# yabebalFantaye/MCEvidence

Hardware: AMD Instinct MI355X
Metric: knn_queries_per_sec (higher is better)
Workload: dtype f16 filter + f64 refine (exact f64 results)

## Files before the change

mcevidence_amd/csrc/capi_common.hpp:

```cpp
#pragma once
namespace {

thread_local char g_err[512] = "";
thread_local char g_last_kernel[256] = "";
thread_local int g_prof_on = 0;
thread_local std::vector<std::pair<hipEvent_t, hipEvent_t>> g_ev_pool;
thread_local size_t g_ev_used = 0;
thread_local size_t g_ev_calls = 0;
thread_local bool g_in_tail = false;
thread_local int g_split_depth = 0;
thread_local double g_last_prune_geom[3] = {0, 0, 0};
thread_local double g_last_flops_main = 0.0, g_last_flops_all = 0.0;
thread_local std::vector<std::pair<hipEvent_t, hipEvent_t>> g_evs_pool;
thread_local size_t g_evs_used = 0;

int fail(int code, const char* fmt, ...)
{
    va_list ap;
    va_start(ap, fmt);
    vsnprintf(g_err, sizeof(g_err), fmt, ap);
    va_end(ap);
    return code;
}

#define MCE_HIP(call)                                                                              \
    do {                                                                                           \
        hipError_t e_ = (call);                                                                    \
        if (e_ != hipSuccess)                                                                      \
            return fail(MCE_ERR_HIP, "%s failed: %s (%s:%d)", #call, hipGetErrorString(e_), __FILE__, __LINE__); \
    } while (0)

std::atomic<int> g_mode{0};
std::atomic<int> g_prune_mode{0};
struct Tuning {
    bool sym_kernel_f16 = false, tail_split = true, prune_prof = false, wide = true;
    int spin_limit = 1 << 21, sym_bucket = 0, sym_panel = 0, sym_seed_rows = 0, sym_seed_share = 2, sym_seed_mode = -1;
    int f16_seed_rows = -1, f16_seed_share = -1, f16_seed_tg = -1, rsplit = 0, panel_debug = 0, sym_chains = 0, panel_qt = 0;
    size_t feed_wave_bytes = 0;
};
Tuning read_tuning()
{
    Tuning t;
    auto num = [](const char* name, int dflt) { const char* e = getenv(name); return e ? atoi(e) : dflt; };
    const char* e = getenv("MCE_SYM_KERNEL");
    t.sym_kernel_f16 = e && strcmp(e, "f16") == 0;
    t.spin_limit = num("MCE_SYM_SPIN_LIMIT", 1 << 21);
    t.sym_bucket = num("MCE_SYM_BUCKET", 0);
    t.sym_panel = num("MCE_SYM_PANEL", 0);
    t.sym_chains = num("MCE_SYM_CHAINS", 0);
    t.sym_seed_rows = num("MCE_SYM_SEED_ROWS", 0);
    t.sym_seed_share = num("MCE_SYM_SEED_SHARE", 2);
    t.sym_seed_mode = num("MCE_SYM_SEED_MODE", -1);
    t.f16_seed_rows = num("MCE_F16_SEED_ROWS", -1);
    t.f16_seed_share = num("MCE_F16_SEED_SHARE", -1);
    t.f16_seed_tg = num("MCE_F16_SEED_TG", -1);
    t.rsplit = num("MCE_RSPLIT", 0);
    t.tail_split = num("MCE_TAIL_SPLIT", 1) != 0;
    t.wide = num("MCE_WIDE", 1) != 0;
    t.panel_debug = num("MCE_PANEL_DEBUG", 0);
    t.panel_qt = num("MCE_PANEL_QT", 0);
    t.prune_prof = getenv("MCE_PRUNE_PROF") != nullptr;
    if ((e = getenv("MCE_FEED_WAVE_BYTES"))) t.feed_wave_bytes = (size_t)std::strtoull(e, nullptr, 10);
    return t;
}
std::atomic<int> g_sym_mode{-1};
int sym_mode()
{
    int m = g_sym_mode.load();
    if (m < 0) {
        const char* e = getenv("MCE_SYM");
        m = e ? atoi(e) : 0;
        if (m < 0 || m > 2) m = 0;
        g_sym_mode.store(m);
    }
    return m;
}
const char* env_prune_heavy() { return getenv("MCE_PRUNE_HEAVY"); }
const char* env_prune_lists() { return getenv("MCE_PRUNE_LISTS"); }
const char* env_prune_times() { return getenv("MCE_PRUNE_TIMES"); }
bool env_long_on() { static const bool v = [] { const char* e = getenv("MCE_LONG"); return !(e && e[0] == '0'); }(); return v; }
bool env_deep_on() { static const bool v = [] { const char* e = getenv("MCE_DEEP"); return !(e && e[0] == '0'); }(); return v; }
int env_feed_eig() { static const int v = [] { const char* e = getenv("MCE_FEED_EIG"); return e && !strcmp(e, "hip") ? 2 : 1; }(); return v; }
bool env_feed_upload_async() { static const bool v = [] { const char* e = getenv("MCE_FEED_UPLOAD"); return e && !strcmp(e, "async"); }(); return v; }
int env_pairs_once_split() { static const int v = [] { const char* e = getenv("MCE_PAIRS_ONCE_SPLIT"); const int n = e ? atoi(e) : 0; return (n >= 1 && n <= 8) ? n : 0; }(); return v; }
int env_pairs_once_panel() { static const int v = [] { const char* e = getenv("MCE_PAIRS_ONCE_PANEL"); const int n = e ? atoi(e) : 0; return n >= 1 ? n : 0; }(); return v; }
struct CallOptions { int search = -1, prune = -1, sym = -1, same_set = -1, verify = -1, eig = 0; };
thread_local CallOptions t_opt;
thread_local std::vector<CallOptions> t_opt_stack;
int eff_search_mode() { return t_opt.search >= 0 ? t_opt.search : g_mode.load(); }
int eff_prune_mode() { return t_opt.prune >= 0 ? t_opt.prune : g_prune_mode.load(); }
int eff_sym_mode() { return t_opt.sym >= 0 ? t_opt.sym : sym_mode(); }
constexpr int kVerifyDefaultRows = 256;
constexpr int64_t kVerifyAlwaysFrom = 65536;
// ... 4 lines not shown
        const char* e = getenv("MCE_VERIFY");
        if (!e || !*e) return kVerifyDefaultRows;
        const long n = strtol(e, nullptr, 10);
        return (int)std::max<long>(0, std::min<long>(n, 1 << 20));
    }();
    return v;
}
bool verify_env_set() { static const bool s = [] { const char* e = getenv("MCE_VERIFY"); return e && *e; }(); return s; }
std::atomic<int> g_last_verify_rows{0};
thread_local unsigned t_small_search_count = 0;
int eff_verify(bool filter_path, int64_t nq)
{
    if (t_opt.verify >= 0) return t_opt.verify;
    if (!filter_path) return 0;
    if (nq < kVerifyAlwaysFrom && !verify_env_set() && (t_small_search_count++ % kVerifySmallEvery) != 0) return 0;
    return default_verify_rows();
}
constexpr int kSymAutoMinBlocks[5] = {0, 768, 257, 193, 193};
constexpr int kSymMaxChains = 8;
constexpr int kSymSeedMode[5] = {0, 0, 1, 1, 1};
constexpr int kSymPartitionMaxParts = 4;
thread_local int g_same_set_hint = -1;
thread_local size_t t_plan_cap = 0;
struct PlanCap {
    size_t prev;
    explicit PlanCap(size_t cap) : prev(t_plan_cap) { t_plan_cap = cap; }
    ~PlanCap() { t_plan_cap = prev; }
};
thread_local bool t_no_heavy = false;
struct NoHeavy {
    bool prev;
    NoHeavy() : prev(t_no_heavy) { t_no_heavy = true; }
    ~NoHeavy() { t_no_heavy = prev; }
};
struct SameSetHint {
    int prev;
    explicit SameSetHint(bool same) : prev(g_same_set_hint) { g_same_set_hint = same ? 1 : 0; }
    ~SameSetHint() { g_same_set_hint = prev; }
};
constexpr int kSymPanelChunks[5] = {0, 96, 256, 256, 256};
int sym_bucket_per_row(int K)
{
    const int b = read_tuning().sym_bucket;
    return b > 0 ? b : 6 * K + 24;
}
constexpr int64_t kPruneAutoMinQueries = 32768;
constexpr int64_t kPruneAutoMinRows[16] = {0, 100000, 100000, 100000, 100000, 125000, 150000, 250000, 500000, 0, 0, 0, 0, 0, 0, 0};

constexpr size_t kPoolMaxBytes = (size_t)64 << 20;
constexpr int kPoolSlots = 16;
struct PoolSlot { void* p = nullptr; size_t cap = 0; int dev = -1; bool busy = false; };
struct Pool {
    PoolSlot slot[kPoolSlots];
    PoolSlot& operator[](int i) { return slot[i]; }
    void release_idle()
    {
        for (int i = 0; i < kPoolSlots; ++i)
            if (slot[i].p && !slot[i].busy) {
                int cur = 0;
                (void)hipGetDevice(&cur);
                if (slot[i].dev != cur) (void)hipSetDevice(slot[i].dev);
                (void)hipFree(slot[i].p);
                if (slot[i].dev != cur) (void)hipSetDevice(cur);
                slot[i] = PoolSlot();
            }
    }
// ... 78 lines not shown
```

mcevidence_amd/csrc/capi_plan.hpp:

```cpp
#pragma once
namespace {

using mce::kMaxDevices;
constexpr int kAssumedCUs = 256;

size_t align_up(size_t x, size_t a) { return (x + a - 1) / a * a; }

constexpr bool kPruneHeavyDefault = false;
constexpr int kPruneHeavyMinBlocks = 64, kPruneHeavyCount = 700, kPruneHeavyMaxShare = 16, kPruneHeavyMinCount = 32, kPruneHeavyMaxRounds = 60;
constexpr double kPruneHeavyFullRounds = 10.0;
constexpr int kPruneHeavySplit = 4, kPruneHeavyMaxSplit = 8;
constexpr int kPruneWaveQueries = mce::kHQT * 32;
constexpr int kPanelWideMinBlocks = 1954;
constexpr int kWideMinBlocks = 480;
bool prune_heavy_enabled()
{
    if (t_no_heavy) return false;
    const char* e = env_prune_heavy();
    return kPruneHeavyDefault || (e && *e && strcmp(e, "0") != 0);
}
static_assert(mce::kPruneWavesPerBlock == mce::kHWaves, "prune.hip orders kHWaves waves per query block");

constexpr int kRefineMargin = 2;
struct Plan {
    const mce::KnnVariant* v = nullptr;
    const mce::KnnF16Variant* vh = nullptr;
    const mce::KnnDeepVariant* vd = nullptr;
    bool filter() const { return vh != nullptr || vd != nullptr; }
    const mce::KnnLongVariant* vl = nullptr;
    size_t off_xf = 0, off_xn = 0;
    bool generic = false;
    int KST = 0;
    size_t off_yh = 0, off_xh = 0, off_qinfo = 0, off_params = 0;
    int KS = 0, KCAP = 0, QT = 0, CT = 0;
    int64_t nchunk = 0;
    int64_t nrow_pad = 0;
    int nqblk = 0;
    int64_t nq_pad = 0;
    int rsplit = 1;
    int L = 4;
    size_t off_yf = 0, off_pd = 0, off_pi = 0, off_center = 0, off_msum = 0, total = 0;
    double cost = 0.0;
    int ksel = 0;
    bool twopass = false;
    bool panel_wide_ok = false;
    bool wide_ok = false;
    bool prune = false;
    bool kd_ready = false;
    int part = 0, nparts = 1;
    int sym_qb_lo = 0, sym_qb_hi = 0;
    bool apo = false;
    int apo_phase = 0;
    int apo_nsplit = 1;
    int apo_panel = 0;
    int64_t pl_nr = 0;
    mce::PruneLayout pl;
    size_t off_prune = 0;
    size_t off_heavy = 0;
    int heavy_max = 0;
    bool sym = false;
    bool sym_active = false;
    mce::SymLayout sl;
    size_t off_sym = 0;
    int sym_nsplit = 1;
    int sym_panel = 0;
};

const mce::KnnVariant* variant_for(int KS, int kcap_idx)
{
    switch (kcap_idx) {
        case 0: return &mce::g_knn_kcap4[mce::mfma_variant_index(KS)];
        case 1: return &mce::g_knn_kcap8[mce::mfma_variant_index(KS)];
        case 2: return &mce::g_knn_kcap12[mce::mfma_variant_index(KS)];
        case 3: return &mce::g_knn_kcap16[mce::mfma_variant_index(KS)];
        case 4: return &mce::g_knn_kcap24[mce::mfma_variant_index(KS)];
        default: return &mce::g_knn_kcap32[mce::mfma_variant_index(KS)];
    }
}

int sweep_seed_cfg(int64_t cps, int CT, int kneed)
{
    const Tuning t = read_tuning();
    if (t.f16_seed_rows >= 0 || t.f16_seed_share >= 0 || t.f16_seed_tg >= 0)
        return mce::f16_seed_cfg(cps, CT, kneed, t.f16_seed_rows >= 0 ? t.f16_seed_rows : MCE_H_SEED_ROWS, t.f16_seed_share >= 0 ? t.f16_seed_share : MCE_H_SEED_SHARE,
                                 t.f16_seed_tg >= 0 ? t.f16_seed_tg : MCE_H_SEED_TG);
    for (int share = MCE_H_SEED_SHARE; share >= 2; share /= 2)
        for (int tg = MCE_H_SEED_TG; tg >= 2; tg /= 2)
            if (const int cfg = mce::f16_seed_cfg(cps, CT, kneed, MCE_H_SEED_ROWS, share, tg)) return cfg;
    return 0;
}

template <class V> const V* by_kcap(int ki, const V* t4, const V* t8, const V* t12, const V* t16) { return ki == 0 ? t4 : ki == 1 ? t8 : ki == 2 ? t12 : t16; }

double split_cost(const Plan& p, bool filt, int64_t nr, int32_t K, int r)
{
    const double n_r = (double)nr / r;
    const double lnf = 1.0 + std::log(std::max(1.0, n_r / K));
    const double block = filt ? 64.0 * p.QT * p.KST * (n_r / 32.0) + 300.0 * 32.0 * p.QT * K * lnf
// ... 174 lines not shown
    p.rsplit = best_r;
    p.cost = split_cost(p, filt, nr, K, best_r);
    auto layout = [&]() {
    p.L = p.twopass ? 2 * p.rsplit : p.rsplit;

    size_t off = 0;
    p.off_yf = off;
    if (filt) {
        p.off_yh = off;
        off = align_up(off + (size_t)p.nrow_pad * (size_t)(16 * p.KST) * 2, 256);
        p.off_xh = off;
        off = align_up(off + (size_t)p.nq_pad * (size_t)(16 * p.KST) * 2, 256);
        p.off_qinfo = off;
        off = align_up(off + (size_t)p.nq_pad * 2 * sizeof(double), 256);
        p.off_params = off;
        off = align_up(off + (size_t)mce::HP_COUNT * sizeof(double), 256);
    } else {
        off = align_up(off + (size_t)p.nrow_pad * (size_t)(4 * p.KS) * sizeof(double), 256);
    }
    if (f16 && (!p.twopass || p.vh->launch_panel_lower) && !p.prune && nq == nr && p.vh->launch_sym && p.nqblk >= 2 && p.nrow_pad <= ((int64_t)1 << mce::kHSymRowBits)) {
        const int sm = eff_sym_mode();
        p.sym = sm == 2 || (sm == 0 && p.nqblk >= kSymAutoMinBlocks[p.KST] * ((p.KST == 1 && p.KCAP == 16) ? 2 : 1));
        if (g_same_set_hint == 0 || (g_same_set_hint < 0 && t_opt.same_set == 0)) p.sym = false;
    }
    p.sym_nsplit = 1;
    p.sym_panel = 0;
    if (p.sym && !p.twopass) {
        const Tuning tun = read_tuning();
        int S = 1;
        if (tun.sym_chains >= 1) S = std::min(tun.sym_chains, kSymMaxChains);
        p.sym_nsplit = S;
        if (S > 1) p.sym_panel = (int)std::max<int64_t>(8, std::min<int64_t>(kSymPanelChunks[p.KST], p.nchunk / (2 * S)));
    }
    const int l_alloc = std::max(p.L, p.sym_nsplit);
    p.off_pd = off;
    off = align_up(off + (size_t)l_alloc * p.KCAP * (size_t)p.nq_pad * sizeof(double), 256);
    p.off_pi = off;
    off = align_up(off + (size_t)l_alloc * p.KCAP * (size_t)p.nq_pad * sizeof(int), 256);
    p.off_center = off;
    off = align_up(off + (size_t)3 * mce::kMaxDimPad * sizeof(double), 256);
    p.off_msum = off;
    off = align_up(off + (size_t)mce::kMeanBlocks * mce::kStatStride * sizeof(double), 256);
    if (p.prune) {
        mce::prune_layout(nq, p.nq_pad, p.nqblk, nr, p.nrow_pad, p.nchunk, d, p.pl);
        p.pl_nr = nr;
        p.off_prune = off;
        off = align_up(off + p.pl.total, 256);
        if (nq == nr && p.nqblk >= kPruneHeavyMinBlocks && prune_heavy_enabled()) {
            p.heavy_max = std::max(p.nqblk * mce::kHWaves / kPruneHeavyMaxShare, kPruneHeavyMinCount);
            p.off_heavy = off;
            off = align_up(off + (size_t)p.heavy_max * kPruneWaveQueries * (kPruneHeavyMaxSplit - 1) * p.KCAP * (sizeof(double) + sizeof(int)), 256);
        }
    }
    if (p.sym) {
        mce::sym_layout(nr, p.nq_pad, p.nqblk, d, p.KCAP, mce::f16_qpb(p.KCAP), sym_bucket_per_row(std::min<int>(K, p.KCAP)), p.sl);
        p.off_sym = off;
        off = align_up(off + p.sl.total, 256);
    }
    p.total = off;
    };
    layout();
    while (t_plan_cap && p.total > t_plan_cap && p.rsplit > std::max(1, rmin)) {
        p.rsplit -= 1;
        layout();
    }
    return MCE_OK;
}

size_t dotp_ws_bytes(int64_t nq, int32_t kmax)
{
    const int64_t nb = (nq + mce::kRedThreads - 1) / mce::kRedThreads;
    return align_up((size_t)std::max<int64_t>(nb, 1) * (size_t)kmax * sizeof(double), 256);
}

int plan_for_workspace(int64_t nq, int64_t nr, int32_t d, int32_t K, int32_t self_mode, size_t ws_bytes, size_t extra, bool same_set_fallback,
                       Plan& p, std::optional<NoHeavy>& nh)
{
    int rc = make_plan(nq, nr, d, K, self_mode, p);
    if (rc != MCE_OK) return rc;
    if (same_set_fallback && ws_bytes < p.total + extra && p.sym) {
        g_same_set_hint = 0;
        rc = make_plan(nq, nr, d, K, self_mode, p);
        if (rc != MCE_OK) return rc;
    }
    if (ws_bytes < p.total + extra && p.heavy_max > 0) {
        nh.emplace();
        rc = make_plan(nq, nr, d, K, self_mode, p);
        if (rc != MCE_OK) return rc;
    }
    if (ws_bytes < p.total + extra) return fail(MCE_ERR_WORKSPACE, "workspace too small: %zu < %zu", ws_bytes, p.total + extra);
    return MCE_OK;
}

}
```

mcevidence_amd/csrc/capi_search.hpp:

```cpp
#pragma once
namespace {

double ln_unit_ball(int d) { return 0.5 * d * std::log(M_PI) - std::lgamma(1.0 + 0.5 * d); }

hipError_t launch_sym_merge(int KCAP, double* pd, int* pi, int64_t nq_pad, const mce::SymParams& sym, int qb_lo, int qb_hi, hipStream_t st, int stride = 1)
{
    const int nb = qb_hi > qb_lo ? (qb_hi - qb_lo + stride - 1) / stride : 0;
    if (nb <= 0) return hipSuccess;
    const dim3 g((unsigned)nb), b(mce::kSymMergeThreads);
    static_assert(mce::kSymMergeThreads == mce::f16_qpb(4), "one merge block per query block");
    switch (KCAP) {
        case 4: hipLaunchKernelGGL(mce::sym_merge_kernel<4>, g, b, 0, st, pd, pi, nq_pad, sym.bucket_cnt, sym.bucket_flag, sym.bucket, sym.cap, qb_lo, stride); break;
        case 8: hipLaunchKernelGGL(mce::sym_merge_kernel<8>, g, b, 0, st, pd, pi, nq_pad, sym.bucket_cnt, sym.bucket_flag, sym.bucket, sym.cap, qb_lo, stride); break;
        case 12: hipLaunchKernelGGL(mce::sym_merge_kernel<12>, g, b, 0, st, pd, pi, nq_pad, sym.bucket_cnt, sym.bucket_flag, sym.bucket, sym.cap, qb_lo, stride); break;
        default: hipLaunchKernelGGL(mce::sym_merge_kernel<16>, g, b, 0, st, pd, pi, nq_pad, sym.bucket_cnt, sym.bucket_flag, sym.bucket, sym.cap, qb_lo, stride); break;
    }
    return hipGetLastError();
}

struct KernelBracket {
    bool on = false; hipStream_t st = nullptr;
    hipError_t begin() const
    {
        if (!on) return hipSuccess;
// ... 269 lines not shown
    mce::knn_f16_launch_fn short_fn = nullptr;
    int short_lc = 0;
    if (p.vh->launch_prune_short && K <= p.vh->prune_short_lc) { short_fn = p.vh->launch_prune_short; short_lc = p.vh->prune_short_lc; }
    else if (p.vh->launch_prune_short2 && K <= p.vh->prune_short_lc2) { short_fn = p.vh->launch_prune_short2; short_lc = p.vh->prune_short_lc2; }
    const bool short_lists = short_fn && !(force_lists && !strcmp(force_lists, "long"));
    MCE_HIP(short_lists ? short_fn(a, st) : p.vh->launch_prune(a, st));
    MCE_HIP(kb.end());
    if (a.wg_us) {
        std::vector<float> us(n_wg);
        MCE_HIP(hipStreamSynchronize(st));
        MCE_HIP(hipMemcpy(us.data(), a.wg_us, n_wg * sizeof(float), hipMemcpyDeviceToHost));
        if (FILE* fh = fopen(times_file, "wb")) {
            const int hdr[4] = {(int)n_wg, hv_n, hv_S, 1};
            fwrite(hdr, sizeof(int), 4, fh);
            fwrite(us.data(), sizeof(float), n_wg, fh);
            fclose(fh);
        }
    }
    if (hv_n) {
        const unsigned fb = (unsigned)(((int64_t)hv_n * kPruneWaveQueries + mce::kRedThreads - 1) / mce::kRedThreads);
        hipLaunchKernelGGL(mce::prune_heavy_fold_kernel, dim3(fb), dim3(mce::kRedThreads), 0, st, pd, pi, p.nq_pad, p.KCAP, hv_d, hv_i, hv_n, hv_S,
                           kPruneWaveQueries, po.border, a.qblk0, a.qblk_stride);
        MCE_HIP(hipGetLastError());
    }
    g_last_params = a.params;
    g_last_flops_main = g_last_flops_all = -1.0;
    g_last_prune_geom[0] = p.nqblk; g_last_prune_geom[1] = (double)p.nchunk; g_last_prune_geom[2] = p.CT;
    snprintf(g_last_kernel, sizeof(g_last_kernel), "%s pruned grid=%d block=64 lds=%zu qt=%d ct=%d chunks=%lld heavy=%dx%d lists=%d", p.vh->name,
             nblk_run + hv_n * (hv_S - 1), mce::f16_prune_lds_bytes(p.KST, d, short_lists ? short_lc : p.KCAP), p.QT, p.CT, (long long)p.nchunk, hv_n,
             hv_S, short_lists ? short_lc : p.KCAP);
    return MCE_OK;
}

int sym_units_and_flops(const Plan& p, const mce::PanelGeom& g, bool panel_kernel, int64_t nr, int panel)
{
    int units = mce::sym_unit_count(p.nqblk, mce::kHWaves * mce::kHQT, panel * p.CT, (int)((nr + 31) / 32) + (int)(((nr + 31) / 32) & 1));
    double tiles = 0.0;
    double qtiles = 16.0;
    if (panel_kernel) {
        units = mce::panel_unit_count(g);
        qtiles = g.tpb;
        for (int u = 0; g_prof_on && u < units; ++u) {
            int pp, aa, lo, hi;
            mce::panel_unit_decode(u, g, pp, aa);
            mce::panel_unit_tiles(pp, aa, g, lo, hi);
            tiles += hi - lo;
        }
    } else {
        const double tpb = mce::kHWaves * mce::kHQT, T = (double)((nr + 31) / 32);
        for (int b = 0; b < p.nqblk; ++b) tiles += std::min(tpb * (b + 1), T);
    }
    g_last_flops_main = tiles * qtiles * 1024.0 * 32.0 * p.KST;
    return units;
}

int Search::symmetric()
{
    char* const sw = ws + p.off_sym;
    mce::KnnF16Args a = sym_args(p, ws, nr, d, K, self_exclude);
    const Tuning tun = read_tuning();
    const int seed_rows = tun.sym_seed_rows > 0 ? tun.sym_seed_rows : (p.KST == 1 ? 65536 : 32768) * (p.apo && p.nparts >= 4 ? 2 : 1);
    const int seed_share = tun.sym_seed_share;
    auto sym_seed_for = [&](int kk) {
        int cfg = mce::f16_seed_cfg(p.nchunk, p.CT, kk + a.self_exclude, seed_rows, seed_share, MCE_H_SEED_TG);
        for (int tg = MCE_H_SEED_TG / 2; cfg == 0 && tg >= 1; tg /= 2)
            cfg = mce::f16_seed_cfg(p.nchunk, p.CT, kk + a.self_exclude, seed_rows, seed_share, tg);
        if (cfg) cfg |= ((tun.sym_seed_mode >= 0 ? tun.sym_seed_mode : kSymSeedMode[p.KST]) & 3) << 28;
        return cfg;
    };
    const int qb_lo = p.nparts > 1 && !p.apo ? (int)((int64_t)p.nqblk * p.part / p.nparts) : 0;
    const int qb_hi = p.nparts > 1 && !p.apo ? (int)((int64_t)p.nqblk * (p.part + 1) / p.nparts) : p.nqblk;
    p.sym_qb_lo = qb_lo; p.sym_qb_hi = qb_hi;
    const bool panel_kernel = !tun.sym_kernel_f16 || p.nparts > 1 || p.twopass;
    mce::PanelGeom geom;
    geom.qb_lo = qb_lo; geom.qb_hi = qb_hi; geom.tpb = mce::kHWaves * mce::kHQT; geom.ct = p.CT; geom.tpp = a.sym.panel * p.CT; geom.sym_on = 1;
    geom.ntiles = (int)((nr + 31) / 32) + (int)(((nr + 31) / 32) & 1);
    const bool apo = p.apo && p.nparts > 1 && !p.twopass && panel_kernel;
    const bool chains1 = !apo && p.nparts == 1 && panel_kernel && !p.twopass && p.sym_nsplit > 1;
    if (apo) { geom.blk_first = p.part; geom.blk_stride = p.nparts; }
    if (apo || chains1) {
        const int pn = apo ? p.apo_panel : p.sym_panel;
        if (pn > 0 && (apo || tun.sym_panel <= 0)) { a.sym.panel = pn; geom.tpp = a.sym.panel * p.CT; }
        geom.nsplit = std::max(1, apo ? p.apo_nsplit : p.sym_nsplit);
        if (geom.nsplit > 1) {
            a.sym.done = reinterpret_cast<int*>(sw + p.sl.keys_b);
            MCE_HIP(mce::zero_async(a.sym.done, (size_t)p.nqblk * geom.nsplit * sizeof(int), st));
            if (!apo) {
                hipLaunchKernelGGL(mce::sym_chain_init_kernel, dim3((unsigned)p.nqblk), dim3(512), 0, st, pd, pi, p.nq_pad, p.KCAP, geom.nsplit, 0, 1);
                MCE_HIP(hipGetLastError());
            }
        }
    }
    const bool unit_table = apo || geom.nsplit > 1;
    const bool panel_wide = panel_kernel && p.panel_wide_ok && p.nparts == 1 && !p.twopass && !unit_table &&
                            (tun.panel_qt == 4 || (tun.panel_qt != 2 && p.nqblk >= kPanelWideMinBlocks));
    if (panel_wide) { geom.tpb = 2 * mce::kHWaves * mce::kHQT; geom.qb_lo = 0; geom.qb_hi = (p.nqblk + 1) / 2; }
    const int npass = p.twopass ? 2 : 1;
    int seed_used = 0;
    for (int pass = 0; pass < npass; ++pass) {
        const bool lower = pass == 1;
        const int Kp = !p.twopass ? K : (lower ? K - 16 : 16);
        double* const pdp = pd + (lower ? list_set(p, 1) : 0);
        int* const pip = pi + (lower ? list_set(p, 1) : 0);
        if (lower) {
            MCE_HIP(mce::zero_async(a.sym.bucket_cnt, (size_t)3 * p.nqblk * sizeof(int), st));
            a.sym.slot_stride = p.KCAP;
        }
        a.ksel = lower ? K : Kp;
        a.seed_cfg = sym_seed_for(a.ksel);
        a.part_d = pdp; a.part_i = pip;
        a.qblk0 = qb_lo;
        a.nqblk_run = qb_hi - qb_lo;
        if (apo) {
            a.qblk0 = p.part; a.qblk_stride = p.nparts; a.nqblk_run = mce::apo_rank_count(p.nqblk, p.part, p.nparts);
        }
        if (a.nqblk_run > 0 && phase != 2) MCE_HIP((lower ? p.vh->launch_sym_pre32 : p.vh->launch_sym_pre)(a, st));
        a.qblk0 = 0; a.qblk_stride = 1; a.nqblk_run = 0;
        if (phase == 1) return MCE_OK;
        if (pass == 0) seed_used = a.seed_cfg;
        a.seed_cfg = 0;
        a.ksel = Kp;
        a.lo_d = lower ? pd : nullptr; a.lo_i = lower ? pi : nullptr;
        if (pass == 0) MCE_HIP(kb.begin());
        if (panel_kernel) {
            mce::PanelArgs pa;
            pa.Yh = static_cast<const _Float16*>(a.Yh); pa.Xh = static_cast<const _Float16*>(a.Xh); pa.qinfo = a.qinfo; pa.params = a.params;
            pa.X = a.X; pa.Y = a.Y; pa.rperm = a.rperm;
            pa.part_d = pdp; pa.part_i = pip; pa.nq = nq; pa.nr = nr; pa.nq_pad = p.nq_pad; pa.self_offset = 0;
            pa.D = d; pa.ksel = Kp; pa.self_exclude = a.self_exclude; pa.spin_limit = tun.spin_limit;
            pa.sym = a.sym; pa.debug = tun.panel_debug; pa.geom = geom; pa.lo_d = a.lo_d; pa.lo_i = a.lo_i;
            if (unit_table) {
                const int nun = mce::panel_unit_count(geom);
                if ((size_t)nun * sizeof(mce::PanelUnit) > (size_t)p.nq_pad * sizeof(int)) return fail(MCE_ERR_INVALID, "symmetric sweep: %d units do not fit the table", nun);
                mce::PanelUnit* tab = reinterpret_cast<mce::PanelUnit*>(sw + p.sl.vals_a);
                if (nun > 0) {
                    hipLaunchKernelGGL(mce::panel_unit_table_kernel, dim3((unsigned)((nun + 255) / 256)), dim3(256), 0, st, geom, nun, tab);
                    MCE_HIP(hipGetLastError());
                }
                pa.units = tab;
            }
            MCE_HIP((lower ? p.vh->launch_panel_lower : (panel_wide ? p.vh->launch_panel_wide : p.vh->launch_panel))(pa, st));
        } else {
            MCE_HIP(p.vh->launch_sym(a, st));
        }
        if (pass == 0) MCE_HIP(kb.end());
        if (apo) break;
        MCE_HIP((lower ? p.vh->launch_sym_repair_lower : p.vh->launch_sym_repair)(a, st));
        if (geom.nsplit > 1) {
            hipLaunchKernelGGL(mce::sym_chain_clear_kernel, dim3((unsigned)p.nqblk), dim3(512), 0, st, a.sym.bucket_flag, pdp, pip, p.nq_pad, p.KCAP, geom.nsplit, 0, 1);
            MCE_HIP(hipGetLastError());
        }
        MCE_HIP(launch_sym_merge(p.KCAP, pdp, pip, p.nq_pad, a.sym, qb_lo, qb_hi, st));
    }
    p.sym_active = true;
    p.L = geom.nsplit > 1 ? geom.nsplit : npass;
    const int sym_units = sym_units_and_flops(p, geom, panel_kernel, nr, a.sym.panel);
    g_last_flops_all = g_last_flops_main + (double)(seed_used & 0xffff) * p.CT * (double)(qb_hi - qb_lo) * 16.0 * 1024.0 * 32.0 * p.KST;
    snprintf(g_last_kernel, sizeof(g_last_kernel), "%s symmetric%s%s%s grid=%d block=%d lds=%zu qt=%d ct=%d panel=%d seed=%dx%d/%d bucket=%d", p.vh->name, panel_kernel ? " panel-kernel" : "",
             p.twopass ? " two passes" : "", geom.blk_stride > 1 ? " pairs-once" : (geom.nsplit > 1 ? " chains" : ""), sym_units,
             mce::kHThreads, panel_wide ? p.vh->lds_bytes_panel_wide : (panel_kernel ? p.vh->lds_bytes_panel : p.vh->lds_bytes_sym), panel_wide ? 2 * p.QT : p.QT, p.CT, a.sym.panel, seed_used & 0xffff, (seed_used >> 16) & 0xfff, (seed_used >> 28) & 3, p.sl.cap);
    return MCE_OK;
}

int Search::f16_sweep(const F16Search& f)
{
    mce::KnnF16Args a = f16_args(p, ws, f.sX, nq, f.sY, nr, d, K, self_exclude, self_offset);
    auto seed_cfg = [&](int ksel) { return sweep_seed_cfg(p.nchunk / p.rsplit, p.CT, ksel + a.self_exclude); };
    MCE_HIP(kb.begin());
    if (p.twopass) {
        a.ksel = 16;
        a.seed_cfg = seed_cfg(16);
        MCE_HIP(p.vh->launch(a, st));
        a.lo_d = pd; a.lo_i = pi;
        a.part_d = pd + list_set(p, p.rsplit); a.part_i = pi + list_set(p, p.rsplit);
        a.ksel = K - 16;
        a.seed_cfg = 0;
        MCE_HIP(p.vh->launch_lower(a, st));
    } else {
        a.seed_cfg = seed_cfg(K);
        if (p.wide_ok) MCE_HIP(p.vh->launch_wide(a, st));
        else MCE_HIP(p.vh->launch(a, st));
    }
    MCE_HIP(kb.end());
    const int seed_first = p.twopass ? seed_cfg(16) : a.seed_cfg;
    g_last_flops_main = (double)p.nqblk * ((double)p.nchunk + (double)(seed_first & 0xffff) * p.rsplit) * p.CT * 16.0 * 1024.0 * 32.0 * p.KST +
                        (p.twopass ? (double)p.nqblk * (double)p.nchunk * p.CT * 16.0 * 1024.0 * 32.0 * p.KST : 0.0);
    g_last_flops_all = g_last_flops_main;
    char seed_txt[48] = "";
    if (seed_first) snprintf(seed_txt, sizeof(seed_txt), " seed=%dx%d", seed_first & 0xffff, seed_first >> 16);
    const bool wide = p.wide_ok && !p.twopass;
    snprintf(g_last_kernel, sizeof(g_last_kernel), "%s grid=%d block=%d lds=%zu qt=%d ct=%d rsplit=%d%s%s%s", p.vh->name,
             (wide ? p.nqblk / 2 : p.nqblk) * p.rsplit, mce::kHThreads, wide ? p.vh->lds_bytes_wide : p.vh->lds_bytes, wide ? 2 * p.QT : p.QT, p.CT, p.rsplit,
             p.twopass ? " two passes" : "", seed_txt, wide ? " wide" : "");
// ... 116 lines not shown
```

mcevidence_amd/csrc/knn_inst.hip:

```cpp
#include "knn_mfma.hpp"
#include "knn_f16.hpp"
#include "knn_panel.hpp"
#include "knn_deep.hpp"
#include "knn_dispatch.hpp"

#ifndef MCE_KCAP
#error "compile with -DMCE_KCAP=n"
#endif
#ifndef MCE_INST_PART
#define MCE_INST_PART 0
#endif
#define MCE_INST_F16 (MCE_KCAP <= 16 && (MCE_INST_PART == 0 || MCE_INST_PART == 1))
#define MCE_INST_F64 (MCE_INST_PART == 0 || MCE_INST_PART == 2)
#define MCE_INST_PANEL (MCE_KCAP <= 16 && (MCE_INST_PART == 0 || MCE_INST_PART == 3))
#define MCE_INST_DEEP (MCE_KCAP <= 16 && (MCE_INST_PART == 0 || MCE_INST_PART == 4))

namespace mce {

#if MCE_INST_F64
template <int KS, int KCAP>
hipError_t launch_variant(const KnnArgs& a, hipStream_t st)
{
    constexpr size_t LDS = lds_bytes(KS, KCAP);
    static_assert(LDS <= 160 * 1024, "LDS budget");
// ... 29 lines not shown
        hipError_t e = hipFuncSetAttribute(reinterpret_cast<const void*>(kern), hipFuncAttributeMaxDynamicSharedMemorySize, (int)LDS_MAX);
        if (e != hipSuccess) return e;
        if (dev < kMaxDevices) attr_set[dev] = true;
    }
    const int ntiles_even = (int)((a.nr + 31) / 32) + (int)(((a.nr + 31) / 32) & 1);
    const int hv_n = PRUNE ? (a.seed_cfg & 0xffffff) : 0, hv_S = PRUNE && ((a.seed_cfg >> 24) & 0x7f) > 1 ? ((a.seed_cfg >> 24) & 0x7f) : 1;
    const dim3 grid((unsigned)(PRUNE ? (a.nqblk_run ? a.nqblk_run : a.nqblk * kHWaves) + hv_n * (hv_S - 1)
                               : SYM == 2 ? sym_unit_count(a.nqblk, kHWaves * kHQT, a.sym.panel * f16_chunk_tiles(KST), ntiles_even)
                               : SYM == 1 ? (a.nqblk_run ? a.nqblk_run : a.nqblk) : (a.nqblk / WB) * a.rsplit));
    hipLaunchKernelGGL(kern, grid, dim3(PRUNE ? 64 : kHThreads), LDS, st, static_cast<const _Float16*>(a.Yh), a.nchunk_total, a.rsplit,
                       static_cast<const _Float16*>(a.Xh), a.qinfo, a.params, a.X, a.Y, a.nq, a.nr, a.D, a.nq_pad, a.nqblk / WB,
                       a.self_exclude, a.self_offset, a.ksel, a.part_d, a.part_i, a.clist, a.cdist, a.list_len, a.rperm, a.qperm, a.tbox_r, a.tbox_q, a.cbox_r, a.qblk0, a.qblk_stride, a.border, a.lo_d, a.lo_i, a.seed_cfg, a.sym, a.wg_us);
    return hipGetLastError();
}
#endif

#if MCE_INST_F16 || MCE_INST_PANEL
template <int KST, int KCAP, bool LOWER = false, int QT = 2>
hipError_t launch_panel_variant(const PanelArgs& a, hipStream_t st)
#if MCE_INST_PANEL
{
    constexpr size_t LDS = panel_lds_bytes(KST, QT);
    static_assert(LDS <= 160 * 1024, "LDS budget");
    static bool attr_set[kMaxDevices] = {};
    auto kern = knn_panel_kernel<KST, KCAP, LOWER, QT>;
    int dev = 0;
    (void)hipGetDevice(&dev);
    if (dev >= kMaxDevices || !attr_set[dev]) {
        hipError_t e = hipFuncSetAttribute(reinterpret_cast<const void*>(kern), hipFuncAttributeMaxDynamicSharedMemorySize, (int)LDS);
        if (e != hipSuccess) return e;
        if (dev < kMaxDevices) attr_set[dev] = true;
    }
    if (a.geom.tpb != 8 * QT) return hipErrorInvalidValue;
    const int units = panel_unit_count(a.geom);
    if (units <= 0) return hipSuccess;
    hipLaunchKernelGGL(kern, dim3((unsigned)units), dim3(kHThreads), LDS, st, a);
    return hipGetLastError();
}
template hipError_t launch_panel_variant<1, MCE_KCAP>(const PanelArgs&, hipStream_t);
template hipError_t launch_panel_variant<2, MCE_KCAP>(const PanelArgs&, hipStream_t);
template hipError_t launch_panel_variant<3, MCE_KCAP>(const PanelArgs&, hipStream_t);
template hipError_t launch_panel_variant<4, MCE_KCAP>(const PanelArgs&, hipStream_t);
template hipError_t launch_panel_variant<1, MCE_KCAP, false, 4>(const PanelArgs&, hipStream_t);
template hipError_t launch_panel_variant<2, MCE_KCAP, false, 4>(const PanelArgs&, hipStream_t);
#if MCE_KCAP == 16
template hipError_t launch_panel_variant<1, MCE_KCAP, true>(const PanelArgs&, hipStream_t);
template hipError_t launch_panel_variant<2, MCE_KCAP, true>(const PanelArgs&, hipStream_t);
template hipError_t launch_panel_variant<3, MCE_KCAP, true>(const PanelArgs&, hipStream_t);
template hipError_t launch_panel_variant<4, MCE_KCAP, true>(const PanelArgs&, hipStream_t);
#endif
#else
;
extern template hipError_t launch_panel_variant<1, MCE_KCAP>(const PanelArgs&, hipStream_t);
extern template hipError_t launch_panel_variant<2, MCE_KCAP>(const PanelArgs&, hipStream_t);
extern template hipError_t launch_panel_variant<3, MCE_KCAP>(const PanelArgs&, hipStream_t);
extern template hipError_t launch_panel_variant<4, MCE_KCAP>(const PanelArgs&, hipStream_t);
extern template hipError_t launch_panel_variant<1, MCE_KCAP, false, 4>(const PanelArgs&, hipStream_t);
extern template hipError_t launch_panel_variant<2, MCE_KCAP, false, 4>(const PanelArgs&, hipStream_t);
#if MCE_KCAP == 16
extern template hipError_t launch_panel_variant<1, MCE_KCAP, true>(const PanelArgs&, hipStream_t);
extern template hipError_t launch_panel_variant<2, MCE_KCAP, true>(const PanelArgs&, hipStream_t);
extern template hipError_t launch_panel_variant<3, MCE_KCAP, true>(const PanelArgs&, hipStream_t);
extern template hipError_t launch_panel_variant<4, MCE_KCAP, true>(const PanelArgs&, hipStream_t);
#endif
#endif
#endif

// ... 132 lines not shown
```

mcevidence_amd/csrc/sym_exchange.hpp:

```cpp
#pragma once
#include <hip/hip_runtime.h>
#include <stdint.h>

#include "sym_types.hpp"

namespace mce {

constexpr int kApoScanThreads = 256;

MCE_HD inline int apo_rank_count(int nqblk, int s, int W) { return s < nqblk ? (nqblk - s + W - 1) / W : 0; }
MCE_HD inline int apo_rank_base(int nqblk, int s, int W) { const int q = nqblk / W, rem = nqblk % W; return s * q + (s < rem ? s : rem); }
MCE_HD inline int apo_block_at(int nqblk, int v, int W)
{
    const int q = nqblk / W, rem = nqblk % W;
    if (v < rem * (q + 1)) return v / (q + 1) + W * (v % (q + 1));
    const int v2 = v - rem * (q + 1);
    return rem + v2 / q + W * (v2 % q);
}

__global__ __launch_bounds__(kApoScanThreads) void apo_offsets_kernel(const int* __restrict__ bucket_cnt, int* __restrict__ bucket_flag, int cap, int nqblk,
                                                                       int part, int nparts, int* __restrict__ offs, long long* __restrict__ counts,
                                                                       int* __restrict__ flags_out)
{
    __shared__ int part_sum[kApoScanThreads];
// ... 61 lines not shown
    const int run_end = above ? __builtin_ctzll(above) : 64;
    int base = 0;
    if (lane == run_start && jb >= 0) base = atomicAdd(bucket_cnt + jb, run_end - run_start);
    base = __shfl(base, run_start, 64);
    if (jb < 0) return;
    const int slot = base + (lane - run_start);
    if ((unsigned)slot < (unsigned)cap) bucket[(int64_t)jb * cap + slot] = e;
    else bucket_flag[jb] = 1;
}

__global__ __launch_bounds__(256) void apo_flags_kernel(const int* __restrict__ flags_all, int* __restrict__ bucket_flag, int nqblk, int part, int nparts)
{
    const int b = part + nparts * (blockIdx.x * 256 + threadIdx.x);
    if (b < nqblk && flags_all[b] != 0) bucket_flag[b] = 1;
}

__global__ __launch_bounds__(256) void panel_unit_table_kernel(PanelGeom g, int nunits, PanelUnit* __restrict__ out)
{
    const int u = blockIdx.x * 256 + threadIdx.x;
    if (u >= nunits) return;
    int p, a, lo, hi;
    panel_unit_decode(u, g, p, a);
    panel_unit_tiles(p, a, g, lo, hi);
    const int S = g.nsplit > 1 ? g.nsplit : 1;
    PanelUnit t;
    t.qblk = a; t.t_lo = lo; t.t_hi = hi;
    t.useq = S > 1 ? p / S : panel_unit_seq(p, a, g);
    t.chain = S > 1 ? a * S + p % S : a;
    t.list_set = S > 1 ? p % S : 0;
    t.pad0 = t.pad1 = 0;
    out[u] = t;
}

__global__ __launch_bounds__(512) void sym_chain_init_kernel(double* __restrict__ pd, int* __restrict__ pi, int64_t nq_pad, int KCAP, int S, int part, int nparts)
{
    const int64_t q = (int64_t)(part + nparts * (int)blockIdx.x) * 512 + threadIdx.x;
    for (int s = 0; s < S; ++s)
        for (int k = 0; k < KCAP; ++k) {
            const int64_t o = ((int64_t)s * KCAP + k) * nq_pad + q;
            pd[o] = __builtin_huge_val();
            pi[o] = -1;
        }
}
__global__ __launch_bounds__(512) void sym_chain_clear_kernel(const int* __restrict__ bucket_flag, double* __restrict__ pd, int* __restrict__ pi, int64_t nq_pad, int KCAP,
                                                              int S, int part, int nparts)
{
    const int b = part + nparts * (int)blockIdx.x;
    if (bucket_flag[b] == 0) return;
    const int64_t q = (int64_t)b * 512 + threadIdx.x;
    for (int s = 1; s < S; ++s)
        for (int k = 0; k < KCAP; ++k) {
            const int64_t o = ((int64_t)s * KCAP + k) * nq_pad + q;
            pd[o] = __builtin_huge_val();
            pi[o] = -1;
        }
}

__global__ __launch_bounds__(256) void apo_iota_kernel(int* __restrict__ out, int n)
{
    const int i = blockIdx.x * 256 + threadIdx.x;
    if (i < n) out[i] = i;
}

}
```

mcevidence_amd/csrc/sym_types.hpp:

```cpp
#pragma once
#include <stdint.h>

namespace mce {

struct SymEntry { double d2; int src; int row; };
struct SymParams {
    unsigned long long* thr = nullptr;
    unsigned* rrow = nullptr;
    float* rtile = nullptr;
    unsigned long long* slots = nullptr;
    int* bucket_cnt = nullptr;
    int* bucket_flag = nullptr;
    SymEntry* bucket = nullptr;
    int cap = 0;
    int* done = nullptr;
    int panel = 0;
    int slot_stride = 0;
};

#if defined(__HIPCC__)
#define MCE_HD __host__ __device__
#else
#define MCE_HD
#endif

MCE_HD inline int sym_unit_count(int nqblk, int tpb, int tpp, int ntiles)
{
    int total = 0;
    for (int p = 0; (int64_t)p * tpp < ntiles; ++p) total += nqblk - (int)(((int64_t)p * tpp) / tpb);
    return total;
}
MCE_HD inline void sym_unit_decode(int u, int nqblk, int tpb, int tpp, int& p, int& a)
{
    for (p = 0;; ++p) {
        const int amin = (int)(((int64_t)p * tpp) / tpb);
        const int cnt = nqblk - amin;
        if (u < cnt) { a = nqblk - 1 - u; return; }
        u -= cnt;
    }
}
MCE_HD inline void sym_unit_tiles(int p, int a, int tpb, int tpp, int ntiles, int& lo, int& hi)
{
    const int hi_a = tpb * (a + 1) < ntiles ? tpb * (a + 1) : ntiles;
    lo = p * tpp;
    hi = (p + 1) * tpp < hi_a ? (p + 1) * tpp : hi_a;
}

struct PanelUnit { int qblk, t_lo, t_hi, useq, chain, list_set, pad0, pad1; };
struct PanelGeom {
    int qb_lo = 0, qb_hi = 0;
    int tpb = 16;
    int tpp = 0;
    int ct = 0;
    int ntiles = 0;
    int sym_on = 0;
    int blk_first = 0, blk_stride = 0;
    int nsplit = 1;
};
MCE_HD inline int panel_r1(const PanelGeom& g) { return g.sym_on ? (g.tpb * g.qb_hi < g.ntiles ? g.tpb * g.qb_hi : g.ntiles) : g.ntiles; }
MCE_HD inline int panel_r2(const PanelGeom& g) { return g.sym_on ? g.tpb * g.qb_hi : g.ntiles; }
MCE_HD inline int panel_r2c(const PanelGeom& g) { return panel_r2(g) / g.ct * g.ct; }
MCE_HD inline int panel_n1(const PanelGeom& g) { return (panel_r1(g) + g.tpp - 1) / g.tpp; }
MCE_HD inline int panel_n2(const PanelGeom& g) { return panel_r2(g) < g.ntiles ? (g.ntiles - panel_r2c(g) + g.tpp - 1) / g.tpp : 0; }
MCE_HD inline int panel_hi_a(const PanelGeom& g, int a)
{
    const int r1 = panel_r1(g);
    return g.sym_on ? (g.tpb * (a + 1) < r1 ? g.tpb * (a + 1) : r1) : r1;
}
MCE_HD inline int panel_amin(const PanelGeom& g, int p)
{
    if (!g.sym_on || p >= panel_n1(g)) return g.qb_lo;
    const int amin = (int)(((int64_t)p * g.tpp) / g.tpb);
    return amin > g.qb_lo ? amin : g.qb_lo;
}
MCE_HD inline int panel_nown(const PanelGeom& g, int amin)
{
    if (g.blk_stride <= 1) return g.qb_hi - amin;
    const int total = g.qb_hi > g.blk_first ? (g.qb_hi - g.blk_first + g.blk_stride - 1) / g.blk_stride : 0;
    const int skip = amin <= g.blk_first ? 0 : (amin - g.blk_first + g.blk_stride - 1) / g.blk_stride;
    return total > skip ? total - skip : 0;
}
MCE_HD inline int panel_unit_count(const PanelGeom& g)
{
    int total = 0;
    const int np = panel_n1(g) + panel_n2(g);
    for (int p = 0; p < np; ++p) total += panel_nown(g, panel_amin(g, p));
    return total;
}
MCE_HD inline void panel_unit_decode(int u, const PanelGeom& g, int& p, int& a)
{
    for (p = 0;; ++p) {
        const int cnt = panel_nown(g, panel_amin(g, p));
        if (u < cnt) {
            a = g.blk_stride <= 1 ? g.qb_hi - 1 - u : g.blk_first + g.blk_stride * (panel_nown(g, 0) - 1 - u);
            return;
        }
        u -= cnt;
    }
}
MCE_HD inline void panel_unit_tiles(int p, int a, const PanelGeom& g, int& lo, int& hi)
{
    const int n1 = panel_n1(g);
    if (p < n1) {
        const int hi_a = panel_hi_a(g, a);
        lo = p * g.tpp;
        hi = (p + 1) * g.tpp < hi_a ? (p + 1) * g.tpp : hi_a;
    } else {
        const int r2 = panel_r2(g), r2c = panel_r2c(g), k = p - n1;
        lo = k == 0 ? r2 : r2c + k * g.tpp;
        hi = r2c + (k + 1) * g.tpp < g.ntiles ? r2c + (k + 1) * g.tpp : g.ntiles;
    }
}
MCE_HD inline int panel_unit_seq(int p, int a, const PanelGeom& g)
{
    const int n1 = panel_n1(g);
    if (p < n1) return p;
    return (panel_hi_a(g, a) + g.tpp - 1) / g.tpp + (p - n1);
}

}
```

Before: 28.16 million.

## Split underfilled tail panels of wide symmetric sweep into parallel partial-list chains

For the wide symmetric panel kernel, panels whose owned-unit count is below the device CU count are split into several tile-range parts. Each part writes to its own partial top-K list set and chain, and the repair/merge step combines them. The aim is to fill idle CUs during the triangular tail, where few work units remain. In exchange it needs extra workspace for the additional list sets, plus init and table kernels. The wide-panel threshold is also lowered so the wide form applies to more problem sizes.

```diff
diff --git a/mcevidence_amd/csrc/capi_common.hpp b/mcevidence_amd/csrc/capi_common.hpp
--- a/mcevidence_amd/csrc/capi_common.hpp
+++ b/mcevidence_amd/csrc/capi_common.hpp
@@ -36,6 +36,7 @@
     bool sym_kernel_f16 = false, tail_split = true, prune_prof = false, wide = true;
     int spin_limit = 1 << 21, sym_bucket = 0, sym_panel = 0, sym_seed_rows = 0, sym_seed_share = 2, sym_seed_mode = -1;
     int f16_seed_rows = -1, f16_seed_share = -1, f16_seed_tg = -1, rsplit = 0, panel_debug = 0, sym_chains = 0, panel_qt = 0;
+    int panel_tail = -1, panel_tail_w = 0, panel_tail_min = 0;
     size_t feed_wave_bytes = 0;
 };
 Tuning read_tuning()
@@ -59,6 +60,9 @@
     t.wide = num("MCE_WIDE", 1) != 0;
     t.panel_debug = num("MCE_PANEL_DEBUG", 0);
     t.panel_qt = num("MCE_PANEL_QT", 0);
+    t.panel_tail = num("MCE_PANEL_TAIL", -1);
+    t.panel_tail_w = num("MCE_PANEL_TAIL_W", 0);
+    t.panel_tail_min = num("MCE_PANEL_TAIL_MIN", 0);
     t.prune_prof = getenv("MCE_PRUNE_PROF") != nullptr;
     if ((e = getenv("MCE_FEED_WAVE_BYTES"))) t.feed_wave_bytes = (size_t)std::strtoull(e, nullptr, 10);
     return t;
@@ -129,6 +133,12 @@
     bool prev;
     NoHeavy() : prev(t_no_heavy) { t_no_heavy = true; }
     ~NoHeavy() { t_no_heavy = prev; }
+};
+thread_local bool t_no_panel_tail = false;
+struct NoPanelTail {
+    bool prev;
+    NoPanelTail() : prev(t_no_panel_tail) { t_no_panel_tail = true; }
+    ~NoPanelTail() { t_no_panel_tail = prev; }
 };
 struct SameSetHint {
     int prev;
diff --git a/mcevidence_amd/csrc/capi_plan.hpp b/mcevidence_amd/csrc/capi_plan.hpp
--- a/mcevidence_amd/csrc/capi_plan.hpp
+++ b/mcevidence_amd/csrc/capi_plan.hpp
@@ -11,7 +11,10 @@
 constexpr double kPruneHeavyFullRounds = 10.0;
 constexpr int kPruneHeavySplit = 4, kPruneHeavyMaxSplit = 8;
 constexpr int kPruneWaveQueries = mce::kHQT * 32;
-constexpr int kPanelWideMinBlocks = 1954;
+constexpr int kPanelWideMinBlocks = 1024;
+constexpr int kPanelTailParts = 2;
+constexpr int kPanelTailMaxParts = 4;
+constexpr int kPanelTailMinChunks = 8;
 constexpr int kWideMinBlocks = 480;
 bool prune_heavy_enabled()
 {
@@ -64,6 +67,7 @@
     size_t off_sym = 0;
     int sym_nsplit = 1;
     int sym_panel = 0;
+    int panel_tail = 1;
 };
 
 const mce::KnnVariant* variant_for(int KS, int kcap_idx)
@@ -304,7 +308,14 @@
         p.sym_nsplit = S;
         if (S > 1) p.sym_panel = (int)std::max<int64_t>(8, std::min<int64_t>(kSymPanelChunks[p.KST], p.nchunk / (2 * S)));
     }
-    const int l_alloc = std::max(p.L, p.sym_nsplit);
+    p.panel_tail = 1;
+    if (p.sym && !p.twopass && p.panel_wide_ok && p.sym_nsplit == 1 && !t_no_panel_tail) {
+        const Tuning tun = read_tuning();
+        const int S = tun.panel_tail >= 0 ? tun.panel_tail : kPanelTailParts;
+        const bool wide_form = !tun.sym_kernel_f16 && (tun.panel_qt == 4 || (tun.panel_qt != 2 && p.nqblk >= kPanelWideMinBlocks));
+        if (wide_form && S >= 2) p.panel_tail = std::min(S, kPanelTailMaxParts);
+    }
+    const int l_alloc = std::max(std::max(p.L, p.sym_nsplit), p.panel_tail);
     p.off_pd = off;
     off = align_up(off + (size_t)l_alloc * p.KCAP * (size_t)p.nq_pad * sizeof(double), 256);
     p.off_pi = off;
@@ -350,6 +361,11 @@
 {
     int rc = make_plan(nq, nr, d, K, self_mode, p);
     if (rc != MCE_OK) return rc;
+    if (ws_bytes < p.total + extra && p.panel_tail > 1) {
+        NoPanelTail nt;
+        rc = make_plan(nq, nr, d, K, self_mode, p);
+        if (rc != MCE_OK) return rc;
+    }
     if (same_set_fallback && ws_bytes < p.total + extra && p.sym) {
         g_same_set_hint = 0;
         rc = make_plan(nq, nr, d, K, self_mode, p);
diff --git a/mcevidence_amd/csrc/capi_search.hpp b/mcevidence_amd/csrc/capi_search.hpp
--- a/mcevidence_amd/csrc/capi_search.hpp
+++ b/mcevidence_amd/csrc/capi_search.hpp
@@ -325,6 +325,19 @@
     return MCE_OK;
 }
 
+int device_cu_count()
+{
+    static std::atomic<int> cus[kMaxDevices] = {};
+    int dev = 0;
+    (void)hipGetDevice(&dev);
+    int n = dev >= 0 && dev < kMaxDevices ? cus[dev].load() : 0;
+    if (n <= 0) {
+        if (hipDeviceGetAttribute(&n, hipDeviceAttributeMultiprocessorCount, dev) != hipSuccess || n <= 0) n = kAssumedCUs;
+        if (dev >= 0 && dev < kMaxDevices) cus[dev].store(n);
+    }
+    return n;
+}
+
 int sym_units_and_flops(const Plan& p, const mce::PanelGeom& g, bool panel_kernel, int64_t nr, int panel)
 {
     int units = mce::sym_unit_count(p.nqblk, mce::kHWaves * mce::kHQT, panel * p.CT, (int)((nr + 31) / 32) + (int)(((nr + 31) / 32) & 1));
@@ -332,6 +345,7 @@
     double qtiles = 16.0;
     if (panel_kernel) {
         units = mce::panel_unit_count(g);
+        const int launched = g.tail_s > 1 ? mce::panel_tail_unit_count(g) : units;
         qtiles = g.tpb;
         for (int u = 0; g_prof_on && u < units; ++u) {
             int pp, aa, lo, hi;
@@ -339,6 +353,7 @@
             mce::panel_unit_tiles(pp, aa, g, lo, hi);
             tiles += hi - lo;
         }
+        units = launched;
     } else {
         const double tpb = mce::kHWaves * mce::kHQT, T = (double)((nr + 31) / 32);
         for (int b = 0; b < p.nqblk; ++b) tiles += std::min(tpb * (b + 1), T);
@@ -388,6 +403,21 @@
     const bool panel_wide = panel_kernel && p.panel_wide_ok && p.nparts == 1 && !p.twopass && !unit_table &&
                             (tun.panel_qt == 4 || (tun.panel_qt != 2 && p.nqblk >= kPanelWideMinBlocks));
     if (panel_wide) { geom.tpb = 2 * mce::kHWaves * mce::kHQT; geom.qb_lo = 0; geom.qb_hi = (p.nqblk + 1) / 2; }
+    int tail_cut = 0;
+    if (panel_wide && p.panel_tail > 1) {
+        geom.tail_s = p.panel_tail;
+        geom.tail_w = tun.panel_tail_w > 0 ? tun.panel_tail_w : device_cu_count();
+        geom.tail_min = tun.panel_tail_min > 0 ? tun.panel_tail_min : kPanelTailMinChunks;
+        mce::panel_tail_unit_count(geom, &tail_cut);
+        if (tail_cut == 0) { geom.tail_s = 1; geom.tail_w = 0; geom.tail_min = 1; }
+    }
+    const bool tail_table = geom.tail_s > 1;
+    if (tail_table) {
+        a.sym.done = reinterpret_cast<int*>(sw + p.sl.keys_b);
+        MCE_HIP(mce::zero_async(a.sym.done, (size_t)geom.qb_hi * geom.tail_s * sizeof(int), st));
+        hipLaunchKernelGGL(mce::panel_tail_init_kernel, dim3((unsigned)p.nqblk), dim3(512), 0, st, pd, pi, p.nq_pad, p.KCAP, geom.tail_s);
+        MCE_HIP(hipGetLastError());
+    }
     const int npass = p.twopass ? 2 : 1;
     int seed_used = 0;
     for (int pass = 0; pass < npass; ++pass) {
@@ -422,12 +452,13 @@
             pa.part_d = pdp; pa.part_i = pip; pa.nq = nq; pa.nr = nr; pa.nq_pad = p.nq_pad; pa.self_offset = 0;
             pa.D = d; pa.ksel = Kp; pa.self_exclude = a.self_exclude; pa.spin_limit = tun.spin_limit;
             pa.sym = a.sym; pa.debug = tun.panel_debug; pa.geom = geom; pa.lo_d = a.lo_d; pa.lo_i = a.lo_i;
-            if (unit_table) {
-                const int nun = mce::panel_unit_count(geom);
+            if (unit_table || tail_table) {
+                const int nun = tail_table ? mce::panel_tail_unit_count(geom) : mce::panel_unit_count(geom);
                 if ((size_t)nun * sizeof(mce::PanelUnit) > (size_t)p.nq_pad * sizeof(int)) return fail(MCE_ERR_INVALID, "symmetric sweep: %d units do not fit the table", nun);
                 mce::PanelUnit* tab = reinterpret_cast<mce::PanelUnit*>(sw + p.sl.vals_a);
                 if (nun > 0) {
-                    hipLaunchKernelGGL(mce::panel_unit_table_kernel, dim3((unsigned)((nun + 255) / 256)), dim3(256), 0, st, geom, nun, tab);
+                    if (tail_table) hipLaunchKernelGGL(mce::panel_tail_table_kernel, dim3((unsigned)((nun + 255) / 256)), dim3(256), 0, st, geom, nun, tab);
+                    else hipLaunchKernelGGL(mce::panel_unit_table_kernel, dim3((unsigned)((nun + 255) / 256)), dim3(256), 0, st, geom, nun, tab);
                     MCE_HIP(hipGetLastError());
                 }
                 pa.units = tab;
@@ -439,19 +470,22 @@
         if (pass == 0) MCE_HIP(kb.end());
         if (apo) break;
         MCE_HIP((lower ? p.vh->launch_sym_repair_lower : p.vh->launch_sym_repair)(a, st));
-        if (geom.nsplit > 1) {
-            hipLaunchKernelGGL(mce::sym_chain_clear_kernel, dim3((unsigned)p.nqblk), dim3(512), 0, st, a.sym.bucket_flag, pdp, pip, p.nq_pad, p.KCAP, geom.nsplit, 0, 1);
+        if (geom.nsplit > 1 || tail_table) {
+            hipLaunchKernelGGL(mce::sym_chain_clear_kernel, dim3((unsigned)p.nqblk), dim3(512), 0, st, a.sym.bucket_flag, pdp, pip, p.nq_pad, p.KCAP,
+                               tail_table ? geom.tail_s : geom.nsplit, 0, 1);
             MCE_HIP(hipGetLastError());
         }
         MCE_HIP(launch_sym_merge(p.KCAP, pdp, pip, p.nq_pad, a.sym, qb_lo, qb_hi, st));
     }
     p.sym_active = true;
-    p.L = geom.nsplit > 1 ? geom.nsplit : npass;
+    p.L = geom.nsplit > 1 ? geom.nsplit : (tail_table ? geom.tail_s : npass);
     const int sym_units = sym_units_and_flops(p, geom, panel_kernel, nr, a.sym.panel);
+    char tail_word[32] = "";
+    if (tail_table) snprintf(tail_word, sizeof(tail_word), " tail=%dx%d", geom.tail_s, tail_cut);
     g_last_flops_all = g_last_flops_main + (double)(seed_used & 0xffff) * p.CT * (double)(qb_hi - qb_lo) * 16.0 * 1024.0 * 32.0 * p.KST;
-    snprintf(g_last_kernel, sizeof(g_last_kernel), "%s symmetric%s%s%s grid=%d block=%d lds=%zu qt=%d ct=%d panel=%d seed=%dx%d/%d bucket=%d", p.vh->name, panel_kernel ? " panel-kernel" : "",
+    snprintf(g_last_kernel, sizeof(g_last_kernel), "%s symmetric%s%s%s grid=%d block=%d lds=%zu qt=%d ct=%d panel=%d seed=%dx%d/%d bucket=%d%s", p.vh->name, panel_kernel ? " panel-kernel" : "",
              p.twopass ? " two passes" : "", geom.blk_stride > 1 ? " pairs-once" : (geom.nsplit > 1 ? " chains" : ""), sym_units,
-             mce::kHThreads, panel_wide ? p.vh->lds_bytes_panel_wide : (panel_kernel ? p.vh->lds_bytes_panel : p.vh->lds_bytes_sym), panel_wide ? 2 * p.QT : p.QT, p.CT, a.sym.panel, seed_used & 0xffff, (seed_used >> 16) & 0xfff, (seed_used >> 28) & 3, p.sl.cap);
+             mce::kHThreads, panel_wide ? p.vh->lds_bytes_panel_wide : (panel_kernel ? p.vh->lds_bytes_panel : p.vh->lds_bytes_sym), panel_wide ? 2 * p.QT : p.QT, p.CT, a.sym.panel, seed_used & 0xffff, (seed_used >> 16) & 0xfff, (seed_used >> 28) & 3, p.sl.cap, tail_word);
     return MCE_OK;
 }
 
diff --git a/mcevidence_amd/csrc/knn_inst.hip b/mcevidence_amd/csrc/knn_inst.hip
--- a/mcevidence_amd/csrc/knn_inst.hip
+++ b/mcevidence_amd/csrc/knn_inst.hip
@@ -85,7 +85,8 @@
         if (dev < kMaxDevices) attr_set[dev] = true;
     }
     if (a.geom.tpb != 8 * QT) return hipErrorInvalidValue;
-    const int units = panel_unit_count(a.geom);
+    const int units = a.geom.tail_s > 1 ? panel_tail_unit_count(a.geom) : panel_unit_count(a.geom);
+    if (a.geom.tail_s > 1 && !a.units) return hipErrorInvalidValue;
     if (units <= 0) return hipSuccess;
     hipLaunchKernelGGL(kern, dim3((unsigned)units), dim3(kHThreads), LDS, st, a);
     return hipGetLastError();
diff --git a/mcevidence_amd/csrc/sym_exchange.hpp b/mcevidence_amd/csrc/sym_exchange.hpp
--- a/mcevidence_amd/csrc/sym_exchange.hpp
+++ b/mcevidence_amd/csrc/sym_exchange.hpp
@@ -117,6 +117,22 @@
     out[u] = t;
 }
 
+__global__ __launch_bounds__(256) void panel_tail_table_kernel(PanelGeom g, int nunits, PanelUnit* __restrict__ out)
+{
+    const int u = blockIdx.x * 256 + threadIdx.x;
+    if (u < nunits) out[u] = panel_tail_unit(u, g);
+}
+__global__ __launch_bounds__(512) void panel_tail_init_kernel(double* __restrict__ pd, int* __restrict__ pi, int64_t nq_pad, int KCAP, int S)
+{
+    const int64_t q = (int64_t)blockIdx.x * 512 + threadIdx.x;
+    for (int s = 1; s < S; ++s)
+        for (int k = 0; k < KCAP; ++k) {
+            const int64_t o = ((int64_t)s * KCAP + k) * nq_pad + q;
+            pd[o] = __builtin_huge_val();
+            pi[o] = -1;
+        }
+}
+
 __global__ __launch_bounds__(512) void sym_chain_init_kernel(double* __restrict__ pd, int* __restrict__ pi, int64_t nq_pad, int KCAP, int S, int part, int nparts)
 {
     const int64_t q = (int64_t)(part + nparts * (int)blockIdx.x) * 512 + threadIdx.x;
diff --git a/mcevidence_amd/csrc/sym_types.hpp b/mcevidence_amd/csrc/sym_types.hpp
--- a/mcevidence_amd/csrc/sym_types.hpp
+++ b/mcevidence_amd/csrc/sym_types.hpp
@@ -56,6 +56,9 @@
     int sym_on = 0;
     int blk_first = 0, blk_stride = 0;
     int nsplit = 1;
+    int tail_s = 1;
+    int tail_w = 0;
+    int tail_min = 1;
 };
 MCE_HD inline int panel_r1(const PanelGeom& g) { return g.sym_on ? (g.tpb * g.qb_hi < g.ntiles ? g.tpb * g.qb_hi : g.ntiles) : g.ntiles; }
 MCE_HD inline int panel_r2(const PanelGeom& g) { return g.sym_on ? g.tpb * g.qb_hi : g.ntiles; }
@@ -118,4 +121,83 @@
     return (panel_hi_a(g, a) + g.tpp - 1) / g.tpp + (p - n1);
 }
 
-}
+MCE_HD inline bool panel_tail_panel(const PanelGeom& g, int p)
+{
+    return g.tail_s > 1 && g.sym_on && p < panel_n1(g) && panel_nown(g, panel_amin(g, p)) < g.tail_w;
+}
+MCE_HD inline int panel_tail_chunks(const PanelGeom& g, int p, int a)
+{
+    int lo, hi;
+    panel_unit_tiles(p, a, g, lo, hi);
+    return (hi - lo + g.ct - 1) / g.ct;
+}
+MCE_HD inline int panel_tail_parts(const PanelGeom& g, int p, int a)
+{
+    if (!panel_tail_panel(g, p)) return 1;
+    const int64_t need = (int64_t)g.tail_s * (g.tail_min > 1 ? g.tail_min : 1);
+    return panel_tail_chunks(g, p, a) >= need ? g.tail_s : 1;
+}
+MCE_HD inline void panel_tail_part_tiles(const PanelGeom& g, int p, int a, int s, int& lo, int& hi)
+{
+    int ulo, uhi;
+    panel_unit_tiles(p, a, g, ulo, uhi);
+    const int S = panel_tail_parts(g, p, a);
+    const int nch = (uhi - ulo + g.ct - 1) / g.ct;
+    lo = ulo + (int)((int64_t)s * nch / S) * g.ct;
+    hi = ulo + (int)((int64_t)(s + 1) * nch / S) * g.ct;
+    if (hi > uhi) hi = uhi;
+}
+MCE_HD inline int panel_tail_unit_count(const PanelGeom& g, int* nsplit_units = nullptr)
+{
+    int total = 0, cut = 0;
+    const int np = panel_n1(g) + panel_n2(g);
+    for (int p = 0; p < np; ++p) {
+        const int amin = panel_amin(g, p);
+        if (!panel_tail_panel(g, p)) { total += panel_nown(g, amin); continue; }
+        for (int a = g.qb_hi - 1; a >= amin; --a) {
+            const int n = panel_tail_parts(g, p, a);
+            total += n;
+            cut += n > 1;
+        }
+    }
+    if (nsplit_units) *nsplit_units = cut;
+    return total;
+}
+MCE_HD inline void panel_tail_decode(int u, const PanelGeom& g, int& p, int& a, int& s)
+{
+    for (p = 0;; ++p) {
+        const int amin = panel_amin(g, p);
+        if (!panel_tail_panel(g, p)) {
+            const int cnt = panel_nown(g, amin);
+            if (u < cnt) { a = g.qb_hi - 1 - u; s = 0; return; }
+            u -= cnt;
+            continue;
+        }
+        for (a = g.qb_hi - 1; a >= amin; --a) {
+            const int n = panel_tail_parts(g, p, a);
+            if (u < n) { s = u; return; }
+            u -= n;
+        }
+    }
+}
+MCE_HD inline PanelUnit panel_tail_unit(int u, const PanelGeom& g)
+{
+    int p, a, s;
+    panel_tail_decode(u, g, p, a, s);
+    PanelUnit t;
+    t.qblk = a;
+    panel_tail_part_tiles(g, p, a, s, t.t_lo, t.t_hi);
+    if (s == 0) {
+        t.useq = panel_unit_seq(p, a, g);
+        t.chain = a;
+    } else {
+        t.useq = 0;
+        for (int q = 0; q < p; ++q) t.useq += panel_tail_parts(g, q, a) > 1;
+        t.chain = g.qb_hi * s + a;
+    }
+    t.list_set = s;
+    t.pad0 = t.pad1 = 0;
+    return t;
+}
+
+}
```

Result: no change. 28.33 million, median of 4 (+0.6%).
